# unneon/bioseqdb

Hardware: NVIDIA B200
Metric: 150bp_reads_aligned_per_sec (higher is better)
Workload: dtype int32

## Files before the change

bioseqdb_b200/csrc/finalize.cu:

```cuda
#include "pipeline.cuh"
#include <algorithm>
#include <cstdlib>
#include "ksw_warp.cuh"
#include "ksort_dev.cuh"
#include "launch_cache.cuh"

namespace {

constexpr int FIN_THREADS = 128;
constexpr int FIN_WARPS = FIN_THREADS / 32;
constexpr int NARROW_NC = 64;
constexpr int NARROW_TMAX = 192;
constexpr int NARROW_QMAX = 160;
constexpr int NARROW_THREADS = 128;
constexpr int NARROW_CIG = 48;

struct NarrowJob { uint32_t r, slot; int32_t w2, last_sc, it, score; };

struct FScratch { int* ehh; int* ehe; uint8_t* rseq; uint8_t* query; uint8_t* z; uint32_t* cig; };

__device__ __forceinline__ uint64_t hash_64(uint64_t key) {
    key += ~(key << 32); key ^= (key >> 22); key += ~(key << 13); key ^= (key >> 8);
    key += (key << 3); key ^= (key >> 15); key += ~(key << 27); key ^= (key >> 31);
    return key;
// ... 107 lines not shown
    r = (double)(a.re - b.rb) / (double)(b.re - a.rb) - (double)(a.qe - b.qb) / (double)(b.qe - a.qb);
    r = r > 0. ? r : -r;
    if (a.re < b.rb || a.qe < b.qb) {
        if (w > o.w << 1 || r >= (double)0.05f) return 0;
    } else if (w > o.w << 2 || r >= (double)(0.05f * 2)) return 0;
    w += a.w + b.w;
    w = w < o.w << 2 ? w : o.w << 2;
    GenOut g = gen_cigar2<false>(ix, o, smat, w, b.qe - a.qb, query + a.qb, a.rb, b.re, S, rseq_cap, 0, 0, overflow, need_rseq, cells, calls);
    score = g.score;
    q_s = (int)((double)(b.qe - a.qb) / (double)((b.qe - b.qb) + (a.qe - a.qb)) * (double)(b.score + a.score) + .499);
    r_s = (int)((double)(b.re - a.rb) / (double)((b.re - b.rb) + (a.re - a.rb)) * (double)(b.score + a.score) + .499);
    if ((double)score / (double)(q_s > r_s ? q_s : r_s) < (double)0.90f) return 0;
    *_w = w;
    return score;
}

__device__ __forceinline__ RowDev row_from_reg(const RegRec& ar, const int64_t* ann_id) {
    RowDev row;
    row.rb = ar.rb; row.re = ar.re; row.pos = 0; row.hash = ar.hash; row.qb = ar.qb; row.qe = ar.qe; row.rid = ar.rid; row.score = ar.score;
    row.truesc = ar.truesc; row.sub = ar.sub; row.csub = ar.csub; row.sub_n = ar.sub_n; row.w = ar.w; row.seedcov = ar.seedcov;
    row.secondary = ar.secondary; row.seedlen0 = ar.seedlen0; row.n_comp = ar.n_comp; row.frac_rep = ar.frac_rep;
    row.is_rev = 0; row.mapq = 0;
    row.NM = -1; row.flag = ar.secondary >= 0 ? 0x100 : 0; row.cigar_off = 0; row.n_cigar = 0;
    row.ref_id = ann_id[ar.rid];
    return row;
}

__device__ __forceinline__ int reg2aln_w2(const DevOpts& o, const RegRec& ar) {
    const int qb = ar.qb, qe = ar.qe; const int64_t rb = ar.rb, re = ar.re;
    int tmpw = infer_bw(qe - qb, (int)(re - rb), ar.truesc, o.a, o.o_del, o.e_del);
    int w2 = infer_bw(qe - qb, (int)(re - rb), ar.truesc, o.a, o.o_ins, o.e_ins);
    w2 = w2 > tmpw ? w2 : tmpw;
    if (w2 > o.w) w2 = w2 < ar.w ? w2 : ar.w;
    return w2;
}

__device__ __forceinline__ int gen_cigar_band(const DevOpts& o, int l_query, int rlen, int w_) {
    int max_ins = (int)((double)(((l_query + 1) >> 1) * o.mat[0] - o.o_ins) / o.e_ins + 1.);
    int max_del = (int)((double)(((l_query + 1) >> 1) * o.mat[0] - o.o_del) / o.e_del + 1.);
    int max_gap = max_ins > max_del ? max_ins : max_del;
    max_gap = max_gap > 1 ? max_gap : 1;
    int dl = rlen - l_query; dl = dl < 0 ? -dl : dl;
    int w = (max_gap + dl + 1) >> 1;
    w = w < w_ ? w : w_;
    const int min_w = dl + 3;
    return w > min_w ? w : min_w;
}

constexpr int REG_WT = 16;
constexpr uint32_t NARROW_SHORT_LIST = 1024;
constexpr int REG_WT3 = 8;
constexpr int REG_WT4 = 4;
constexpr int NARROW_T4_CNT = 20, NARROW_T8_CNT = 21;
constexpr int REG_WT2 = 32;
__device__ __forceinline__ bool narrow_is_big(const DevOpts& o, int lq, int rlen, int w2) {
    w2 = w2 < o.w << 2 ? w2 : o.w << 2;
    return gen_cigar_band(o, lq, rlen, w2) > REG_WT;
}
__device__ __forceinline__ bool narrow_is_tight(const DevOpts& o, int lq, int rlen, int wt = REG_WT3) {
    const int dl = lq - rlen;
    return (dl < 0 ? -dl : dl) <= wt && o.o_del >= 0 && o.e_del >= 0 && o.o_ins >= 0 && o.e_ins >= 0 && o.mat_max > 0;
}
__device__ __forceinline__ int narrow_class(const DevOpts& o, const RegRec& ar, uint32_t max_len) {
    const int lq = ar.qe - ar.qb; const int64_t rl = ar.re - ar.rb;
    if (max_len > NARROW_QMAX || lq <= 0 || rl <= 0 || rl > NARROW_TMAX) return 0;
    int w2 = reg2aln_w2(o, ar);
    w2 = w2 < o.w << 2 ? w2 : o.w << 2;
    if (lq == rl) return 2;
    if (2 * gen_cigar_band(o, lq, (int)rl, w2) + 1 <= NARROW_NC) return 1;
    return narrow_is_tight(o, lq, (int)rl) ? 1 : 0;
}
__device__ __forceinline__ void push_narrow(NarrowJob* list, uint32_t cap, uint32_t* cnt_reg, uint32_t* cnt_big, const NarrowJob& jb, bool big) {
    if (big) list[cap - 1u - atomicAdd(cnt_big, 1u)] = jb;
    else list[atomicAdd(cnt_reg, 1u)] = jb;
}

__device__ void reg2aln_warp(const FinalizeParams& P, const DevIndex& ix, const DevOpts& o, const int* smat, const FScratch& S, uint32_t cig_cap,
                             uint32_t rseq_cap, int l_query, const RegRec& ar, RowDev* out, unsigned long long& cells, unsigned long long& calls) {
    const int lane = lane_id();
    const int qb = ar.qb, qe = ar.qe; const int64_t rb = ar.rb, re = ar.re;
    int w2 = reg2aln_w2(o, ar);
    int it = 0, score = 0, last_sc = -(1 << 30);
    GenOut g;
    do {
        w2 = w2 < o.w << 2 ? w2 : o.w << 2;
        g = gen_cigar2<true>(ix, o, smat, w2, qe - qb, S.query + qb, rb, re, S, rseq_cap, P.z_cap, cig_cap - 2, P.overflow, P.need_rseq, cells, calls);
        if (g.ok) score = g.score;
        if (score == last_sc || w2 == o.w << 2) break;
        last_sc = score;
        w2 <<= 1;
    } while (++it < 3 && score < ar.truesc - o.a);
    int is_rev;
    int64_t pos = bns_depos(ix, rb < ix.l_pac ? rb : re - 1, &is_rev);
    int n_cigar = g.n_cigar, first = 0;
    if (n_cigar > 0) {
        if ((S.cig[0] & 0xf) == 2) { pos += S.cig[0] >> 4; first = 1; --n_cigar; }
        else if ((S.cig[g.n_cigar - 1] & 0xf) == 2) --n_cigar;
    }
    int clip5 = 0, clip3 = 0;
    if (qb != 0 || qe != l_query) { clip5 = is_rev ? l_query - qe : qb; clip3 = is_rev ? qb : l_query - qe; }
    const int n_out = n_cigar + (clip5 ? 1 : 0) + (clip3 ? 1 : 0);
    uint32_t coff = 0;
    if (lane == 0 && n_out) coff = atomicAdd(P.cigar_top, (uint32_t)n_out);
    coff = __shfl_sync(FULL, coff, 0);
    uint32_t r_off = 0, r_n = 0;
    if ((uint64_t)coff + (uint64_t)n_out > (uint64_t)P.cigar_cap) { if (lane == 0) atomicExch(P.overflow, 1u); }
// ... 166 lines not shown
            tmp = o.o_ins + o.e_ins > tmp ? o.o_ins + o.e_ins : tmp;
            int nz = 0;
            uint32_t* zl = S.cig;
            zl[nz++] = 0;
            for (int i = 1; i < n; ++i) {
                int k;
                for (k = 0; k < nz; ++k) {
                    const int j = (int)zl[k];
                    const int b_max = a[j].qb > a[i].qb ? a[j].qb : a[i].qb;
                    const int e_min = a[j].qe < a[i].qe ? a[j].qe : a[i].qe;
                    if (e_min > b_max) {
                        const int li = a[i].qe - a[i].qb, lj = a[j].qe - a[j].qb;
                        const int min_l = li < lj ? li : lj;
                        if ((float)(e_min - b_max) >= __fmul_rn((float)min_l, o.mask_level)) {
                            if (a[j].sub == 0) a[j].sub = a[i].score;
                            if (a[j].score - a[i].score <= tmp) ++a[j].sub_n;
                            break;
                        }
                    }
                }
                if (k == nz) { if ((uint32_t)nz < cig_cap) zl[nz] = (uint32_t)i; ++nz; }
                else a[i].secondary = (int)zl[k];
            }
            if ((uint32_t)nz > cig_cap) atomicExch(P.overflow, 2u);
        }
        __syncwarp();
        RowDev* rows = P.rows + blk.base;
        for (int i = 0; i < n; ++i) {
            const RegRec ar = a[i];
            RowDev row = row_from_reg(ar, P.ann_id);
            const int ncls = P.narrow_jobs != nullptr ? narrow_class(o, ar, P.max_len) : 0;
            const bool narrow = ncls != 0;
            if (lane == 0) {
                rows[i] = row;
                if (narrow) {
                    NarrowJob jb; jb.r = r; jb.slot = blk.base + i; jb.w2 = reg2aln_w2(o, ar); jb.last_sc = -(1 << 30); jb.it = 0; jb.score = 0;
                    NarrowJob* lists = reinterpret_cast<NarrowJob*>(P.narrow_jobs);
                    if (ncls == 1 && narrow_is_tight(o, ar.qe - ar.qb, (int)(ar.re - ar.rb))) {
                        if (narrow_is_tight(o, ar.qe - ar.qb, (int)(ar.re - ar.rb), REG_WT4)) lists[3u * P.narrow_cap + atomicAdd(P.narrow_cnt + NARROW_T4_CNT, 1u)] = jb;
                        else lists[4u * P.narrow_cap + atomicAdd(P.narrow_cnt + NARROW_T8_CNT, 1u)] = jb;
                    }
                    else if (ncls == 1) push_narrow(lists, P.narrow_cap, P.narrow_cnt, P.narrow_cnt + 5, jb, narrow_is_big(o, ar.qe - ar.qb, (int)(ar.re - ar.rb), jb.w2));
                    else lists[2u * P.narrow_cap + atomicAdd(P.narrow_cnt + 3, 1u)] = jb;
                }
            }
            __syncwarp();
            if (!narrow) reg2aln_warp(P, ix, o, smat, S, cig_cap, rseq_cap, l_query, ar, rows + i, cells, calls);
        }
        if (lane == 0) P.row_cnt[r] = (uint32_t)n;
    }
    if (P.counters && lane == 0) { atomicAdd(&P.counters[0], cells); atomicAdd(&P.counters[1], calls); }
}

template <int WT, bool TIGHT>
__device__ __forceinline__ int global_dp_reg(const uint8_t* __restrict__ qg, int lq, bool rev, const uint8_t* __restrict__ pac, int64_t tbase,
                                             int rlen, int w, int sA, int sB, int sN, int o_del, int e_del, int o_ins, int e_ins,
                                             uint32_t* __restrict__ Z, unsigned long long& cells, uint32_t* amb_out = nullptr) {
    uint32_t amb = 0;
    constexpr int W = 2 * WT + 1, NW = (W + 7) / 8, ZW = (W + 3) / 4;
    const int oe_del = o_del + e_del, oe_ins = o_ins + e_ins;
    int Hd[W], Ep[W + 1];
    uint32_t win[NW];
#pragma unroll
    for (int kk = 0; kk < W; ++kk) {
        const int j = kk - WT;
        Hd[kk] = (j >= 1 && j <= w) ? -(o_ins + e_ins * j) : KSW_NEG_INF;
        Ep[kk] = KSW_NEG_INF;
    }
    Ep[W] = KSW_NEG_INF;
#pragma unroll
    for (int x = 0; x < NW; ++x) win[x] = 0xffffffffu;
#pragma unroll
    for (int kk = WT; kk < W; ++kk) {
        const int j = kk - WT;
        if (j < lq) {
            const uint32_t b = rev ? qg[lq - 1 - j] : qg[j];
            amb |= b;
            win[kk >> 3] = (win[kk >> 3] & ~(15u << ((kk & 7) * 4))) | (b << ((kk & 7) * 4));
        }
    }
    int tb = rev ? 3 - (int)pac_get(pac, tbase) : (int)pac_get(pac, tbase);
    for (int i = 0; i < rlen; ++i) {
        const int beg = i > w ? i - w : 0;
        const int end = i + w + 1 < lq ? i + w + 1 : lq;
        const int ioff = i - WT - beg;
        const unsigned span = (unsigned)(end - beg);
        const int tz = beg == 0 ? 0 : 0x7fffffff;
        const int colm1 = i == 0 ? 0 : -(o_del + e_del * i);
        cells += span;
        int tb_next = 0; uint32_t nb = 15u;
        if (i + 1 < rlen) tb_next = rev ? 3 - (int)pac_get(pac, tbase + i + 1) : (int)pac_get(pac, tbase + i + 1);
        { const int jn = i + 1 + WT; if (jn < lq) { nb = rev ? qg[lq - 1 - jn] : qg[jn]; amb |= nb; } }
        int f = KSW_NEG_INF;
        uint32_t zpack = 0;
        uint32_t* zi = Z + (size_t)i * ZW * 32;
        if (TIGHT && w == WT && i > WT && i + WT + 1 <= lq) {
            uint32_t xw[NW];
#pragma unroll
            for (int x = 0; x < NW; ++x) xw[x] = win[x] ^ ((uint32_t)tb * 0x11111111u);
#pragma unroll
            for (int kk = 0; kk < W; ++kk) {
                const bool mis = ((xw[kk >> 3] >> ((kk & 7) * 4)) & 15u) != 0;
                const int m = Hd[kk] + (mis ? sB : sA);
                int e = Ep[kk + 1];
                int d = m >= e ? 0 : 1;
                int h = m >= e ? m : e;
// ... 1 lines not shown
                h = h >= f ? h : f;
                Hd[kk] = h;
                int tt = m - oe_del;
                e -= e_del;
                d |= e > tt ? 1 << 2 : 0;
                Ep[kk] = e > tt ? e : tt;
                tt = m - oe_ins;
                f -= e_ins;
                d |= f > tt ? 2 << 4 : 0;
                f = f > tt ? f : tt;
                zpack |= (uint32_t)d << ((kk & 3) * 8);
                if ((kk & 3) == 3 || kk == W - 1) { zi[(kk >> 2) * 32] = zpack; zpack = 0; }
            }
        } else
#pragma unroll
        for (int kk = 0; kk < W; ++kk) {
            const int t = ioff + kk;
            const bool valid = (unsigned)t < span;
            const int qb = (int)((win[kk >> 3] >> ((kk & 7) * 4)) & 15u);
            const int sc = qb == tb ? sA : (qb < 4 ? sB : sN);
            int m = (t == tz ? colm1 : Hd[kk]) + sc;
            int e = Ep[kk + 1];
            int d = m >= e ? 0 : 1;
            int h = m >= e ? m : e;
            d = h >= f ? d : 2;
            h = h >= f ? h : f;
            Hd[kk] = h;
            int tt = m - oe_del;
            e -= e_del;
            d |= e > tt ? 1 << 2 : 0;
            e = e > tt ? e : tt;
            Ep[kk] = valid ? e : KSW_NEG_INF;
            tt = m - oe_ins;
            int f2 = f - e_ins;
            d |= f2 > tt ? 2 << 4 : 0;
            f2 = f2 > tt ? f2 : tt;
            f = valid ? f2 : f;
            zpack |= (uint32_t)d << ((kk & 3) * 8);
            if ((kk & 3) == 3 || kk == W - 1) { zi[(kk >> 2) * 32] = zpack; zpack = 0; }
        }
#pragma unroll
        for (int x = 0; x + 1 < NW; ++x) win[x] = __funnelshift_r(win[x], win[x + 1], 4);
        win[NW - 1] = ((win[NW - 1] >> 4) & ~(15u << (((W - 1) & 7) * 4))) | (nb << (((W - 1) & 7) * 4));
        tb = tb_next;
    }
    const int ks = lq - rlen + WT;
    int score = KSW_NEG_INF;
#pragma unroll
    for (int kk = 0; kk < W; ++kk) if (kk == ks) score = Hd[kk];
    if (TIGHT && amb_out) *amb_out = amb;
    return score;
}

__device__ __forceinline__ uint32_t pac_win16(const uint8_t* pac, int64_t f) {
    const uint32_t* w = reinterpret_cast<const uint32_t*>(pac) + (f >> 4);
    return __funnelshift_l(__byte_perm(w[1], 0, 0x0123), __byte_perm(w[0], 0, 0x0123), (int)(f & 15) << 1);
}
__device__ __forceinline__ int diag_mismatches(const uint8_t* qg, int lq, bool rev, const uint8_t* pac, int64_t tbase, bool* ok) {
    const uint32_t* qa = reinterpret_cast<const uint32_t*>(reinterpret_cast<uintptr_t>(qg) & ~(uintptr_t)3);
    const int sh = (int)(reinterpret_cast<uintptr_t>(qg) & 3) * 8;
    uint32_t prev = qa[0], amb = 0;
    int mm = 0, j0 = 0;
    for (; j0 + 16 <= lq; j0 += 16) {
        uint32_t Q = 0;
#pragma unroll
        for (int k = 0; k < 4; ++k) {
            const uint32_t nx = qa[(j0 >> 2) + k + 1];
            const uint32_t x = __funnelshift_r(prev, nx, sh);
            prev = nx;
            amb |= x;
            Q |= ((x | x >> 6 | x >> 12 | x >> 18) & 0xffu) << (8 * k);
        }
        uint32_t v;
        if (rev) v = ~pac_win16(pac, tbase + lq - 16 - j0);
        else {
            const uint32_t r = __brev(pac_win16(pac, tbase + j0));
            v = ((r >> 1) & 0x55555555u) | ((r & 0x55555555u) << 1);
        }
        const uint32_t d = Q ^ v;
        mm += __popc((d | d >> 1) & 0x55555555u);
    }
    for (int j = j0; j < lq; ++j) {
        const uint32_t q = qg[j];
        amb |= q;
        mm += q != (rev ? 3u - pac_get(pac, tbase + lq - 1 - j) : pac_get(pac, tbase + j));
    }
    *ok = (amb & 0xfcfcfcfcu) == 0;
    return mm;
}

struct NarrowParams {
    const uint8_t* seqs; const uint64_t* offs; const RegRec* regs; RowDev* rows;
    const NarrowJob* jobs; int job_stride; const uint32_t* n_jobs;
    NarrowJob* requeue; uint32_t requeue_cap; uint32_t* requeue_cnt; uint32_t* requeue_big_cnt; uint64_t* wide_jobs; uint32_t* wide_cnt;
    uint32_t* cigar_pool; uint32_t cigar_cap; uint32_t* cigar_top;
    uint8_t* zbuf; uint32_t* ticket; uint32_t* overflow; unsigned long long* counters;
    NarrowJob* tight; uint32_t* tight_cnt;
    uint32_t short_list;
};

template <int MODE>
__global__ void __launch_bounds__(NARROW_THREADS, MODE == 5 ? 10 : (MODE >= 3 ? 6 : (MODE == 1 ? 4 : 2))) regs_cigar_narrow(NarrowParams P, DevIndex ix, DevOpts o) {
    __shared__ int smat[25];
    if (threadIdx.x < 25) smat[threadIdx.x] = o.mat[threadIdx.x];
    __syncthreads();
    const int tid = threadIdx.x, lane = tid & 31;
    const uint32_t gwarp = (blockIdx.x * NARROW_THREADS + tid) >> 5;
    constexpr int WTM = MODE == 2 ? REG_WT2 : (MODE == 3 ? REG_WT3 : (MODE == 4 ? REG_WT4 : REG_WT));
    constexpr int ZROW = (2 * WTM + 1 + 3) / 4;
    uint32_t* Z = reinterpret_cast<uint32_t*>(P.zbuf + (size_t)gwarp * NARROW_TMAX * ZROW * 4 * 32) + lane;
    int oe_del = o.o_del + o.e_del, oe_ins = o.o_ins + o.e_ins, e_del = o.e_del, e_ins = o.e_ins;
    asm volatile("" : "+r"(oe_del), "+r"(oe_ins), "+r"(e_del), "+r"(e_ins));
    const int64_t l_pac = ix.l_pac;
    const uint32_t n_jobs = *P.n_jobs;
    constexpr bool diag_pass = MODE == 5;
    const bool short_list = !diag_pass && n_jobs <= P.short_list;
    unsigned long long cells = 0, calls = 0;
    for (;;) {
        uint32_t t = next_ticket(P.ticket);
        if ((uint64_t)t * 32 >= n_jobs) break;
        const uint32_t j_id = t * 32 + lane;
        uint32_t cg[NARROW_CIG];
        int e_nc = 0, e_first = 0, e_clip5 = 0, e_clip3 = 0, e_n = 0;
        uint32_t e_slot = 0; bool e_on = false;
        if (j_id < n_jobs) {
            const NarrowJob jb = P.jobs[(long)j_id * P.job_stride];
            const uint32_t r = jb.r, slot = jb.slot;
            const uint64_t job = (uint64_t)r << 32 | slot;
            const RegRec ar = P.regs[slot];
            const int l_read = (int)(P.offs[r + 1] - P.offs[r]);
            const int qb = ar.qb, qe = ar.qe, lq = qe - qb;
            const int64_t rb = ar.rb, re = ar.re;
            const int rlen = (int)(re - rb);
            const bool rev = rb >= l_pac;
            const bool reject = lq <= 0 || rb >= re || (rb < l_pac && re > l_pac) || rb < 0 || re > (l_pac << 1);
            const int64_t tbase = rev ? (l_pac << 1) - re : rb;
            const uint8_t* qg = P.seqs + P.offs[r] + qb;
            auto qat = [&](int j) -> int { return (int)(rev ? qg[lq - 1 - j] : qg[j]); };
            int n_cigar = 0, NM = -1, score = jb.score;
            int w2 = jb.w2 < o.w << 2 ? jb.w2 : o.w << 2;
            bool go_wide = false, again = false;
            do {
                n_cigar = 0; NM = -1;
                if (short_list && !reject) { go_wide = true; break; }
                int nm_known = -1;
                if (!reject) {
                    bool diagonal = lq == rlen && w2 == 0;
                    if (diag_pass && lq == rlen) {
                        int sc = 0;
                        bool fast = false;
                        const int mm = diag_mismatches(qg, lq, rev, ix.pac, tbase, &fast);
                        if (fast) { sc = smat[0] * (lq - mm) + smat[1] * mm; nm_known = mm; }
// ... 88 lines not shown
                }
            } while (false);
            if (go_wide) {
                uint32_t k = atomicAdd(P.wide_cnt, 1u);
                P.wide_jobs[k] = job;
            } else if (!again) {
                int is_rev;
                int64_t pos = bns_depos(ix, rb < l_pac ? rb : re - 1, &is_rev);
                int nc = n_cigar, first = 0;
                if (nc > 0) {
                    if ((cg[0] & 0xf) == 2) { pos += cg[0] >> 4; first = 1; --nc; }
                    else if ((cg[n_cigar - 1] & 0xf) == 2) --nc;
                }
                int clip5 = 0, clip3 = 0;
                if (qb != 0 || qe != l_read) { clip5 = is_rev ? l_read - qe : qb; clip3 = is_rev ? qb : l_read - qe; }
                e_nc = nc; e_first = first; e_clip5 = clip5; e_clip3 = clip3; e_n = nc + (clip5 ? 1 : 0) + (clip3 ? 1 : 0);
                e_slot = slot; e_on = true;
                RowDev* out = P.rows + slot;
                const int rid = bns_pos2rid(ix, pos);
                out->NM = NM; out->is_rev = is_rev; out->pos = pos - ix.ann_offset[rid < 0 ? 0 : rid];
            }
        }
        __syncwarp();
        {
            uint32_t incl = (uint32_t)e_n;
#pragma unroll
            for (int d = 1; d < 32; d <<= 1) { const uint32_t up = __shfl_up_sync(FULL, incl, d); if (lane >= d) incl += up; }
            uint32_t base = 0;
            if (lane == 31 && incl) base = atomicAdd(P.cigar_top, incl);
            base = __shfl_sync(FULL, base, 31);
            if (e_on) {
                const uint32_t coff = base + incl - (uint32_t)e_n;
                RowDev* out = P.rows + e_slot;
                if ((uint64_t)coff + (uint64_t)e_n > (uint64_t)P.cigar_cap) { atomicExch(P.overflow, 1u); }
                else {
                    uint32_t* dst = P.cigar_pool + coff;
                    int k = 0;
                    if (e_clip5) dst[k++] = (uint32_t)e_clip5 << 4 | 3;
                    for (int c = 0; c < e_nc; ++c) dst[k++] = cg[e_first + c];
                    if (e_clip3) dst[k++] = (uint32_t)e_clip3 << 4 | 3;
                    out->cigar_off = coff; out->n_cigar = (uint32_t)e_n;
                }
            }
        }
        __syncwarp();
    }
    if (P.counters) {
        cells = __reduce_add_sync(FULL, (unsigned)(cells & 0xffffffffu)) + ((unsigned long long)__reduce_add_sync(FULL, (unsigned)(cells >> 32)) << 32);
        calls = __reduce_add_sync(FULL, (unsigned)calls);
        if (lane == 0) { atomicAdd(&P.counters[0], cells); atomicAdd(&P.counters[1], calls); }
    }
}

template <bool SMEM>
__global__ void __launch_bounds__(FIN_THREADS) regs_cigar_wide(FinalizeParams P, DevIndex ix, DevOpts o, uint32_t cig_cap, uint32_t rseq_cap) {
    extern __shared__ __align__(16) uint8_t dyn_smem[];
    __shared__ int smat[25];
    if (threadIdx.x < 25) smat[threadIdx.x] = o.mat[threadIdx.x];
    __syncthreads();
    const int lane = lane_id();
    const uint32_t gwarp = (blockIdx.x * FIN_THREADS + threadIdx.x) >> 5;
    FScratch S;
    {
        const size_t fast = ((size_t)(P.max_len + 2) * 8 + rseq_cap + P.max_len + 15) & ~(size_t)15;
        uint8_t* gbase = P.scratch + (size_t)gwarp * P.scratch_per_warp;
        uint8_t* fbase = SMEM ? dyn_smem + (size_t)(threadIdx.x >> 5) * fast : gbase;
        S.ehh = reinterpret_cast<int*>(fbase);
        S.ehe = S.ehh + (P.max_len + 2);
        S.rseq = reinterpret_cast<uint8_t*>(S.ehe + (P.max_len + 2));
        S.query = S.rseq + rseq_cap;
        S.cig = reinterpret_cast<uint32_t*>(gbase + fast);
        S.z = reinterpret_cast<uint8_t*>(S.cig + cig_cap);
    }
    unsigned long long cells = 0, calls = 0;
    const uint32_t n_jobs = *P.wide_cnt;
    for (;;) {
        uint32_t t = next_ticket(P.ticket);
        if (t >= n_jobs) break;
        const uint64_t job = P.wide_jobs[t];
        const uint32_t r = (uint32_t)(job >> 32), slot = (uint32_t)job;
        const int l_query = (int)(P.offs[r + 1] - P.offs[r]);
        const uint8_t* qg = P.seqs + P.offs[r];
        for (int i = lane; i < l_query; i += 32) S.query[i] = qg[i];
        __syncwarp();
        const RegRec ar = P.regs[slot];
        reg2aln_warp(P, ix, o, smat, S, cig_cap, rseq_cap, l_query, ar, P.rows + slot, cells, calls);
    }
    if (P.counters && lane == 0) { atomicAdd(&P.counters[0], cells); atomicAdd(&P.counters[1], calls); }
}

}

static size_t fin_fast_bytes(uint32_t max_len, uint32_t rseq_cap) { return ((size_t)(max_len + 2) * 8 + rseq_cap + max_len + 15) & ~(size_t)15; }
static uint32_t fin_cig_cap(uint32_t max_len, uint32_t rseq_cap) { return max_len + rseq_cap + 8; }

size_t finalize_scratch_per_warp(uint32_t max_len, uint32_t rseq_cap, uint32_t* z_cap_out) {
    uint64_t z = (uint64_t)max_len * (uint64_t)rseq_cap;
    const uint64_t z_band = (uint64_t)rseq_cap * 1024;
    if (z > z_band) z = z_band;
    if (z_cap_out) *z_cap_out = (uint32_t)z;
    size_t b = fin_fast_bytes(max_len, rseq_cap) + (size_t)fin_cig_cap(max_len, rseq_cap) * 4 + (size_t)z;
    return (b + 255) & ~(size_t)255;
}

static bool fin_use_smem(uint32_t max_len, uint32_t rseq_cap) { return fin_fast_bytes(max_len, rseq_cap) * FIN_WARPS <= 40 * 1024; }

int finalize_resident_warps() {
    return cached_blocks_per_sm(regs_finalize<false>, FIN_THREADS, 0) * cached_sm_count() * FIN_WARPS;
}

template <int MODE> static int narrow_blocks() { return cached_blocks_per_sm(regs_cigar_narrow<MODE>, NARROW_THREADS, 0) * cached_sm_count(); }
static size_t narrow_z_bytes(int blocks, int wt) { return (size_t)blocks * (NARROW_THREADS / 32) * NARROW_TMAX * ((2 * wt + 1 + 3) / 4) * 4 * 32; }
static size_t narrow_z_front() {
    return std::max(narrow_z_bytes(narrow_blocks<1>(), REG_WT), std::max(narrow_z_bytes(narrow_blocks<3>(), REG_WT3), narrow_z_bytes(narrow_blocks<4>(), REG_WT4)));
}

size_t narrow_zbuf_bytes() { return narrow_z_front() + narrow_z_bytes(narrow_blocks<2>(), REG_WT2); }

void launch_finalize(const FinalizeParams& p, const DevIndex& ix, const DevOpts& o, cudaStream_t st, uint32_t rseq_cap, int n_warps, uint64_t* launches, const ExtAux* aux) {
    const uint32_t cig_cap = fin_cig_cap(p.max_len, rseq_cap);
    int blocks = n_warps / FIN_WARPS;
    if (blocks < 1) blocks = 1;
    const bool smem_ok = fin_use_smem(p.max_len, rseq_cap);
    const size_t smem = smem_ok ? fin_fast_bytes(p.max_len, rseq_cap) * FIN_WARPS : 0;
    if (p.todo && p.narrow_jobs && p.n_reads) {
        regs_finalize_thread<<<(p.n_reads + 127) / 128, 128, 0, st>>>(p, ix, o);
        if (launches) ++*launches;
    }
    if (smem_ok) regs_finalize<true><<<blocks, FIN_THREADS, smem, st>>>(p, ix, o, cig_cap, rseq_cap);
    else regs_finalize<false><<<blocks, FIN_THREADS, 0, st>>>(p, ix, o, cig_cap, rseq_cap);
    if (launches) ++*launches;
    if (!p.narrow_jobs) return;
    {
        NarrowJob* listA = reinterpret_cast<NarrowJob*>(p.narrow_jobs);
        NarrowJob* listB = listA + p.narrow_cap;
        NarrowJob* listS = listA + 2 * (size_t)p.narrow_cap;
        NarrowJob* listT4 = listA + 3 * (size_t)p.narrow_cap;
        NarrowJob* listT8 = listA + 4 * (size_t)p.narrow_cap;
        for (int pass = 0; pass < 4; ++pass) {
            NarrowParams q;
            q.seqs = p.seqs; q.offs = p.offs; q.regs = p.regs; q.rows = p.rows;
            NarrowJob* in = pass == 0 ? listS : (pass == 2 ? listB : listA);
            q.requeue = (pass == 0 || pass == 2) ? listA : listB; q.requeue_cap = p.narrow_cap;
            q.requeue_cnt = p.narrow_cnt + (pass == 0 ? 0 : (pass == 1 ? 1 : (pass == 2 ? 2 : 4)));
            q.requeue_big_cnt = p.narrow_cnt + (pass == 0 ? 5 : (pass == 1 ? 6 : (pass == 2 ? 7 : 4)));
            q.wide_jobs = p.wide_jobs; q.wide_cnt = p.wide_cnt; q.cigar_pool = p.cigar_pool; q.cigar_cap = p.cigar_cap; q.cigar_top = p.cigar_top;
            q.zbuf = p.narrow_z; q.overflow = p.overflow; q.counters = p.counters;
            q.tight = listT4; q.tight_cnt = p.narrow_cnt + NARROW_T4_CNT;
            { static const uint32_t sl = getenv("BSQ_FIN_SHORT_LIST") ? (uint32_t)atoi(getenv("BSQ_FIN_SHORT_LIST")) : NARROW_SHORT_LIST; q.short_list = sl; }
            q.jobs = in; q.job_stride = 1; q.ticket = p.ticket + 1 + pass;
            q.n_jobs = p.narrow_cnt + (pass == 0 ? 3 : (pass == 1 ? 0 : (pass == 2 ? 1 : 2)));
            if (pass == 0) {
                regs_cigar_narrow<5><<<narrow_blocks<5>(), NARROW_THREADS, 0, st>>>(q, ix, o);
                q.jobs = listT4; q.n_jobs = p.narrow_cnt + NARROW_T4_CNT; q.ticket = p.ticket + 9;
                q.tight = listT8; q.tight_cnt = p.narrow_cnt + NARROW_T8_CNT;
                regs_cigar_narrow<4><<<narrow_blocks<4>(), NARROW_THREADS, 0, st>>>(q, ix, o);
                q.jobs = listT8; q.n_jobs = p.narrow_cnt + NARROW_T8_CNT; q.ticket = p.ticket + 10;
                regs_cigar_narrow<3><<<narrow_blocks<3>(), NARROW_THREADS, 0, st>>>(q, ix, o);
                if (launches) *launches += 3;
            } else {
                cudaStream_t s2 = aux ? aux->st[0] : st;
                if (aux) { cudaEventRecord(aux->ev[0], st); cudaStreamWaitEvent(s2, aux->ev[0], 0); }
                regs_cigar_narrow<1><<<narrow_blocks<1>(), NARROW_THREADS, 0, st>>>(q, ix, o);
                q.jobs = in + p.narrow_cap - 1; q.job_stride = -1; q.ticket = p.ticket + 5 + pass;
                q.n_jobs = p.narrow_cnt + (pass == 1 ? 5 : (pass == 2 ? 6 : 7));
                q.zbuf = p.narrow_z + narrow_z_front();
                regs_cigar_narrow<2><<<narrow_blocks<2>(), NARROW_THREADS, 0, s2>>>(q, ix, o);
                if (aux) { cudaEventRecord(aux->ev[1], s2); cudaStreamWaitEvent(st, aux->ev[1], 0); }
                if (launches) *launches += 2;
            }
        }
    }
    {
        FinalizeParams w = p;
        w.ticket = p.ticket + 5;
        if (smem_ok) regs_cigar_wide<true><<<blocks, FIN_THREADS, smem, st>>>(w, ix, o, cig_cap, rseq_cap);
        else regs_cigar_wide<false><<<blocks, FIN_THREADS, 0, st>>>(w, ix, o, cig_cap, rseq_cap);
        if (launches) ++*launches;
    }
}
```

Before: 63.02 million.

## Pack two tight banded DP jobs per thread using 16-bit SIMD lanes

Adds a paired tight-pass kernel in which each thread runs the banded global DP for two jobs at once. The H/E/F values are packed as int16x2 and updated with __viaddmax/__vibmax SIMD intrinsics, and edge rows fall back to a scalar per-half path. The aim is to roughly halve the per-job instruction count in the tight WT=4 and WT=8 passes. In exchange it doubles the traceback buffer per lane, adds a range check that falls back to the old kernel when scores might overflow 16 bits, and adds register pressure plus divergence from mismatched job lengths.

```diff
diff --git a/bioseqdb_b200/csrc/finalize.cu b/bioseqdb_b200/csrc/finalize.cu
--- a/bioseqdb_b200/csrc/finalize.cu
+++ b/bioseqdb_b200/csrc/finalize.cu
@@ -183,6 +183,7 @@
 constexpr int REG_WT3 = 8;
 constexpr int REG_WT4 = 4;
 constexpr int NARROW_T4_CNT = 20, NARROW_T8_CNT = 21;
+constexpr int NARROW_PAIR_CNT = 22;
 constexpr int REG_WT2 = 32;
 __device__ __forceinline__ bool narrow_is_big(const DevOpts& o, int lq, int rlen, int w2) {
     w2 = w2 < o.w << 2 ? w2 : o.w << 2;
@@ -455,6 +456,98 @@
     if (P.counters && lane == 0) { atomicAdd(&P.counters[0], cells); atomicAdd(&P.counters[1], calls); }
 }
 
+template <int WT, bool TIGHT, int ZS>
+__device__ __forceinline__ void dp_row(int (&Hd)[2 * WT + 1], int (&Ep)[2 * WT + 2], const uint32_t (&win)[(2 * WT + 8) / 8], int tb, int i,
+                                       int lq, int w, int sA, int sB, int sN, int o_del, int e_del, int e_ins, int oe_del, int oe_ins, int neg,
+                                       uint32_t* __restrict__ zi, unsigned long long& cells) {
+    constexpr int W = 2 * WT + 1, NW = (W + 7) / 8;
+    const int beg = i > w ? i - w : 0;
+    const int end = i + w + 1 < lq ? i + w + 1 : lq;
+    const int ioff = i - WT - beg;
+    const unsigned span = (unsigned)(end - beg);
+    const int tz = beg == 0 ? 0 : 0x7fffffff;
+    const int colm1 = i == 0 ? 0 : -(o_del + e_del * i);
+    cells += span;
+    int f = neg;
+    uint32_t zpack = 0;
+    if (TIGHT && w == WT && i > WT && i + WT + 1 <= lq) {
+        uint32_t xw[NW];
+#pragma unroll
+        for (int x = 0; x < NW; ++x) xw[x] = win[x] ^ ((uint32_t)tb * 0x11111111u);
+#pragma unroll
+        for (int kk = 0; kk < W; ++kk) {
+            const bool mis = ((xw[kk >> 3] >> ((kk & 7) * 4)) & 15u) != 0;
+            const int m = Hd[kk] + (mis ? sB : sA);
+            int e = Ep[kk + 1];
+            int d = m >= e ? 0 : 1;
+            int h = m >= e ? m : e;
+            d = h >= f ? d : 2;
+            h = h >= f ? h : f;
+            Hd[kk] = h;
+            int tt = m - oe_del;
+            e -= e_del;
+            d |= e > tt ? 1 << 2 : 0;
+            Ep[kk] = e > tt ? e : tt;
+            tt = m - oe_ins;
+            f -= e_ins;
+            d |= f > tt ? 2 << 4 : 0;
+            f = f > tt ? f : tt;
+            zpack |= (uint32_t)d << ((kk & 3) * 8);
+            if ((kk & 3) == 3 || kk == W - 1) { zi[(kk >> 2) * ZS] = zpack; zpack = 0; }
+        }
+    } else
+#pragma unroll
+    for (int kk = 0; kk < W; ++kk) {
+        const int t = ioff + kk;
+        const bool valid = (unsigned)t < span;
+        const int qb = (int)((win[kk >> 3] >> ((kk & 7) * 4)) & 15u);
+        const int sc = qb == tb ? sA : (qb < 4 ? sB : sN);
+        int m = (t == tz ? colm1 : Hd[kk]) + sc;
+        int e = Ep[kk + 1];
+        int d = m >= e ? 0 : 1;
+        int h = m >= e ? m : e;
+        d = h >= f ? d : 2;
+        h = h >= f ? h : f;
+        Hd[kk] = h;
+        int tt = m - oe_del;
+        e -= e_del;
+        d |= e > tt ? 1 << 2 : 0;
+        e = e > tt ? e : tt;
+        Ep[kk] = valid ? e : neg;
+        tt = m - oe_ins;
+        int f2 = f - e_ins;
+        d |= f2 > tt ? 2 << 4 : 0;
+        f2 = f2 > tt ? f2 : tt;
+        f = valid ? f2 : f;
+        zpack |= (uint32_t)d << ((kk & 3) * 8);
+        if ((kk & 3) == 3 || kk == W - 1) { zi[(kk >> 2) * ZS] = zpack; zpack = 0; }
+    }
+}
+
+template <int WT>
+__device__ __forceinline__ void window_init(uint32_t (&win)[(2 * WT + 8) / 8], const uint8_t* __restrict__ qg, int lq, bool rev, uint32_t& amb) {
+    constexpr int W = 2 * WT + 1, NW = (W + 7) / 8;
+#pragma unroll
+    for (int x = 0; x < NW; ++x) win[x] = 0xffffffffu;
+#pragma unroll
+    for (int kk = WT; kk < W; ++kk) {
+        const int j = kk - WT;
+        if (j < lq) {
+            const uint32_t b = rev ? qg[lq - 1 - j] : qg[j];
+            amb |= b;
+            win[kk >> 3] = (win[kk >> 3] & ~(15u << ((kk & 7) * 4))) | (b << ((kk & 7) * 4));
+        }
+    }
+}
+
+template <int WT>
+__device__ __forceinline__ void window_slide(uint32_t (&win)[(2 * WT + 8) / 8], uint32_t nb) {
+    constexpr int W = 2 * WT + 1, NW = (W + 7) / 8;
+#pragma unroll
+    for (int x = 0; x + 1 < NW; ++x) win[x] = __funnelshift_r(win[x], win[x + 1], 4);
+    win[NW - 1] = ((win[NW - 1] >> 4) & ~(15u << (((W - 1) & 7) * 4))) | (nb << (((W - 1) & 7) * 4));
+}
+
 template <int WT, bool TIGHT>
 __device__ __forceinline__ int global_dp_reg(const uint8_t* __restrict__ qg, int lq, bool rev, const uint8_t* __restrict__ pac, int64_t tbase,
                                              int rlen, int w, int sA, int sB, int sN, int o_del, int e_del, int o_ins, int e_ins,
@@ -562,6 +655,133 @@
     return score;
 }
 
+constexpr int PAIR_NEG = -0x4000;
+
+struct DpHalf { const uint8_t* qg; int64_t tbase; int lq, rlen, w; bool rev; };
+
+__device__ __forceinline__ uint32_t prmt(uint32_t a, uint32_t b, uint32_t sel) {
+    uint32_t r;
+    asm("prmt.b32 %0, %1, %2, %3;" : "=r"(r) : "r"(a), "r"(b), "r"(sel));
+    return r;
+}
+__device__ __forceinline__ uint32_t pk2(int v) { return ((uint32_t)v & 0xffffu) * 0x10001u; }
+
+template <int WT>
+__device__ __noinline__ unsigned pair_edge_row(uint32_t* __restrict__ st, int h, const uint32_t (&win)[(2 * WT + 8) / 8], int tb, int i, int lq, int w,
+                                               int sA, int sB, int sN, int o_del, int e_del, int o_ins, int e_ins, uint32_t* __restrict__ zi) {
+    constexpr int W = 2 * WT + 1;
+    const int sh = 16 * h;
+    int H[W], E[W + 1];
+#pragma unroll
+    for (int kk = 0; kk < W; ++kk) { H[kk] = (int16_t)(st[kk] >> sh); E[kk] = (int16_t)(st[W + kk] >> sh); }
+    E[W] = PAIR_NEG;
+    unsigned long long cells = 0;
+    dp_row<WT, true, 64>(H, E, win, tb, i, lq, w, sA, sB, sN, o_del, e_del, e_ins, o_del + e_del, o_ins + e_ins, PAIR_NEG, zi, cells);
+#pragma unroll
+    for (int kk = 0; kk < W; ++kk) {
+        st[kk] = h ? __byte_perm(st[kk], (uint32_t)H[kk], 0x5410) : __byte_perm((uint32_t)H[kk], st[kk], 0x7610);
+        st[W + kk] = h ? __byte_perm(st[W + kk], (uint32_t)E[kk], 0x5410) : __byte_perm((uint32_t)E[kk], st[W + kk], 0x7610);
+    }
+    return (unsigned)cells;
+}
+
+template <int WT>
+__device__ __noinline__ void global_dp_reg_pair(const DpHalf (&hf)[2], const uint8_t* __restrict__ pac, int sA, int sB, int sN, int o_del, int e_del,
+                                                   int o_ins, int e_ins, uint32_t* __restrict__ Z, unsigned long long& cells, int (&score)[2], uint32_t (&amb)[2]) {
+    constexpr int W = 2 * WT + 1, NW = (W + 7) / 8, ZW = (W + 3) / 4;
+    const int oe_del = o_del + e_del, oe_ins = o_ins + e_ins;
+    const uint32_t n_oe_del = pk2(-oe_del), n_oe_ins = pk2(-oe_ins), n_e_del = pk2(-e_del), n_e_ins = pk2(-e_ins), lo = 0x80008000u;
+    const uint32_t t_lo = ((uint32_t)sA & 0xffu) | ((uint32_t)sB & 0xffu) * 0x01010100u, t_hi = ((uint32_t)sB & 0xffu) * 0x01010101u;
+    uint32_t Hd[W], Ep[W + 1];
+    uint32_t win[2][NW];
+    int tb[2];
+#pragma unroll
+    for (int kk = 0; kk < W; ++kk) {
+        const int j = kk - WT;
+        const int a = (j >= 1 && j <= hf[0].w) ? -(o_ins + e_ins * j) : PAIR_NEG, b = (j >= 1 && j <= hf[1].w) ? -(o_ins + e_ins * j) : PAIR_NEG;
+        Hd[kk] = ((uint32_t)a & 0xffffu) | (uint32_t)b << 16;
+        Ep[kk] = pk2(PAIR_NEG);
+    }
+    Ep[W] = pk2(PAIR_NEG);
+#pragma unroll
+    for (int h = 0; h < 2; ++h) {
+        amb[h] = 0; score[h] = KSW_NEG_INF;
+        window_init<WT>(win[h], hf[h].qg, hf[h].rlen > 0 ? hf[h].lq : 0, hf[h].rev, amb[h]);
+        tb[h] = hf[h].rlen > 0 ? (hf[h].rev ? 3 - (int)pac_get(pac, hf[h].tbase) : (int)pac_get(pac, hf[h].tbase)) : 0;
+    }
+    const int rows = hf[0].rlen > hf[1].rlen ? hf[0].rlen : hf[1].rlen;
+    for (int i = 0; i < rows; ++i) {
+        bool live[2], tight[2];
+        int tb_next[2]; uint32_t nb[2];
+#pragma unroll
+        for (int h = 0; h < 2; ++h) {
+            const DpHalf& d = hf[h];
+            live[h] = i < d.rlen;
+            tight[h] = live[h] && d.w == WT && i > WT && i + WT + 1 <= d.lq;
+            tb_next[h] = 0; nb[h] = 15u;
+            if (i + 1 < d.rlen) tb_next[h] = d.rev ? 3 - (int)pac_get(pac, d.tbase + i + 1) : (int)pac_get(pac, d.tbase + i + 1);
+            const int jn = i + 1 + WT;
+            if (live[h] && jn < d.lq) { nb[h] = d.rev ? d.qg[d.lq - 1 - jn] : d.qg[jn]; amb[h] |= nb[h]; }
+        }
+        uint32_t* zi = Z + (size_t)i * ZW * 64;
+        if ((tight[0] || !live[0]) && (tight[1] || !live[1])) {
+            uint32_t sb[2][ZW];
+#pragma unroll
+            for (int h = 0; h < 2; ++h) {
+                uint32_t xw[NW];
+#pragma unroll
+                for (int x = 0; x < NW; ++x) xw[x] = win[h][x] ^ ((uint32_t)tb[h] * 0x11111111u);
+#pragma unroll
+                for (int g = 0; g < ZW; ++g) sb[h][g] = prmt(t_lo, t_hi, (g & 1) ? xw[g >> 1] >> 16 : xw[g >> 1]);
+            }
+            uint32_t f = pk2(PAIR_NEG), za = 0, zb = 0;
+#pragma unroll
+            for (int kk = 0; kk < W; ++kk) {
+                const uint32_t p = (uint32_t)(kk & 3);
+                const uint32_t sc = prmt(sb[0][kk >> 2], sb[1][kk >> 2], p | (p | 8u) << 4 | (p + 4u) << 8 | (p + 12u) << 12);
+                const uint32_t m = __viaddmax_s16x2(Hd[kk], sc, lo);
+                const uint32_t e = Ep[kk + 1];
+                bool mh, ml, fh, fl, eh, el, gh, gl;
+                uint32_t hh = __vibmax_s16x2(m, e, &mh, &ml);
+                hh = __vibmax_s16x2(hh, f, &fh, &fl);
+                Hd[kk] = hh;
+                Ep[kk] = __vibmax_s16x2(__viaddmax_s16x2(m, n_oe_del, lo), __viaddmax_s16x2(e, n_e_del, lo), &eh, &el);
+                f = __vibmax_s16x2(__viaddmax_s16x2(m, n_oe_ins, lo), __viaddmax_s16x2(f, n_e_ins, lo), &gh, &gl);
+                const uint32_t da = (fl ? (ml ? 0u : 1u) : 2u) | (el ? 0u : 4u) | (gl ? 0u : 32u);
+                const uint32_t db = (fh ? (mh ? 0u : 1u) : 2u) | (eh ? 0u : 4u) | (gh ? 0u : 32u);
+                za |= da << ((kk & 3) * 8);
+                zb |= db << ((kk & 3) * 8);
+                if ((kk & 3) == 3 || kk == W - 1) { reinterpret_cast<uint2*>(zi)[(kk >> 2) * 32] = make_uint2(za, zb); za = 0; zb = 0; }
+            }
+            cells += (live[0] ? W : 0) + (live[1] ? W : 0);
+        } else {
+            uint32_t st[2 * W];
+#pragma unroll
+            for (int kk = 0; kk < W; ++kk) { st[kk] = Hd[kk]; st[W + kk] = Ep[kk]; }
+#pragma unroll
+            for (int h = 0; h < 2; ++h) {
+                if (!live[h]) continue;
+                uint32_t wh[NW];
+#pragma unroll
+                for (int x = 0; x < NW; ++x) wh[x] = win[h][x];
+                cells += pair_edge_row<WT>(st, h, wh, tb[h], i, hf[h].lq, hf[h].w, sA, sB, sN, o_del, e_del, o_ins, e_ins, zi + h);
+            }
+#pragma unroll
+            for (int kk = 0; kk < W; ++kk) { Hd[kk] = st[kk]; Ep[kk] = st[W + kk]; }
+        }
+#pragma unroll
+        for (int h = 0; h < 2; ++h) {
+            if (i == hf[h].rlen - 1) {
+                const int ks = hf[h].lq - hf[h].rlen + WT;
+#pragma unroll
+                for (int kk = 0; kk < W; ++kk) if (kk == ks) score[h] = (int16_t)(Hd[kk] >> (16 * h));
+            }
+            if (live[h]) window_slide<WT>(win[h], nb[h]);
+            tb[h] = tb_next[h];
+        }
+    }
+}
+
 __device__ __forceinline__ uint32_t pac_win16(const uint8_t* pac, int64_t f) {
     const uint32_t* w = reinterpret_cast<const uint32_t*>(pac) + (f >> 4);
     return __funnelshift_l(__byte_perm(w[1], 0, 0x0123), __byte_perm(w[0], 0, 0x0123), (int)(f & 15) << 1);
@@ -607,7 +827,178 @@
     uint8_t* zbuf; uint32_t* ticket; uint32_t* overflow; unsigned long long* counters;
     NarrowJob* tight; uint32_t* tight_cnt;
     uint32_t short_list;
+    uint32_t* pair_passes;
 };
+
+__host__ __device__ constexpr int narrow_wt(int mode) { return mode == 2 ? REG_WT2 : (mode == 3 ? REG_WT3 : (mode == 4 ? REG_WT4 : REG_WT)); }
+
+struct NarrowTry {
+    NarrowJob jb; RegRec ar;
+    const uint8_t* qg; int64_t tbase;
+    int l_read, lq, rlen, w2, wx, w, score, n_cigar, NM, nm_known;
+    bool rev, reject, stop, dp, go_wide, again;
+};
+struct PoolEntry { int nc, first, clip5, clip3, n; uint32_t slot; bool on; };
+
+__device__ __forceinline__ int narrow_qat(const NarrowTry& T, int j) { return (int)(T.rev ? T.qg[T.lq - 1 - j] : T.qg[j]); }
+
+template <int MODE>
+__device__ __forceinline__ void narrow_begin(const NarrowParams& P, const DevIndex& ix, const DevOpts& o, const int* smat, bool short_list, int oe_del,
+                                             int oe_ins, const NarrowJob& jb, uint32_t (&cg)[NARROW_CIG], NarrowTry& T) {
+    constexpr bool diag_pass = MODE == 5;
+    constexpr int WTM = narrow_wt(MODE);
+    const int64_t l_pac = ix.l_pac;
+    const uint32_t r = jb.r;
+    T.jb = jb;
+    T.ar = P.regs[jb.slot];
+    T.l_read = (int)(P.offs[r + 1] - P.offs[r]);
+    const int qb = T.ar.qb, lq = T.ar.qe - qb;
+    const int64_t rb = T.ar.rb, re = T.ar.re;
+    const int rlen = (int)(re - rb);
+    T.lq = lq; T.rlen = rlen;
+    T.rev = rb >= l_pac;
+    T.reject = lq <= 0 || rb >= re || (rb < l_pac && re > l_pac) || rb < 0 || re > (l_pac << 1);
+    T.tbase = T.rev ? (l_pac << 1) - re : rb;
+    T.qg = P.seqs + P.offs[r] + qb;
+    T.n_cigar = 0; T.NM = -1; T.score = jb.score; T.nm_known = -1;
+    T.w2 = jb.w2 < o.w << 2 ? jb.w2 : o.w << 2;
+    T.wx = T.w = 0;
+    T.stop = T.dp = T.go_wide = T.again = false;
+    if (short_list && !T.reject) { T.go_wide = true; T.stop = true; return; }
+    if (T.reject) return;
+    bool diagonal = lq == rlen && T.w2 == 0;
+    if (diag_pass && lq == rlen) {
+        int sc = 0;
+        bool fast = false;
+        const int mm = diag_mismatches(T.qg, lq, T.rev, ix.pac, T.tbase, &fast);
+        if (fast) { sc = smat[0] * (lq - mm) + smat[1] * mm; T.nm_known = mm; }
+        else for (int i = 0; i < lq; ++i) {
+            const int tb = T.rev ? 3 - (int)pac_get(ix.pac, T.tbase + i) : (int)pac_get(ix.pac, T.tbase + i);
+            sc += smat[tb * 5 + narrow_qat(T, i)];
+        }
+        if (diagonal || sc > (lq - 1) * o.mat_max - oe_ins - oe_del) { T.score = sc; cg[0] = (uint32_t)lq << 4; T.n_cigar = 1; diagonal = true; }
+        else {
+            if (narrow_is_tight(o, lq, rlen)) P.tight[atomicAdd(P.tight_cnt, 1u)] = jb;
+            else push_narrow(P.requeue, P.requeue_cap, P.requeue_cnt, P.requeue_big_cnt, jb, narrow_is_big(o, lq, rlen, jb.w2));
+            T.again = true; T.stop = true; return;
+        }
+    } else if (diagonal) {
+        int sc = 0;
+        for (int i = 0; i < lq; ++i) {
+            const int tb = T.rev ? 3 - (int)pac_get(ix.pac, T.tbase + i) : (int)pac_get(ix.pac, T.tbase + i);
+            sc += smat[tb * 5 + narrow_qat(T, i)];
+        }
+        T.score = sc; cg[0] = (uint32_t)lq << 4; T.n_cigar = 1;
+    }
+    if (MODE != 5 && !diagonal) {
+        const int wx = gen_cigar_band(o, lq, rlen, T.w2);
+        const int w = MODE >= 3 ? (wx < WTM ? wx : WTM) : wx;
+        T.wx = wx; T.w = w;
+        if (MODE >= 3 && (!narrow_is_tight(o, lq, rlen, WTM) || rlen > NARROW_TMAX)) {
+            push_narrow(P.requeue, P.requeue_cap, P.requeue_cnt, P.requeue_big_cnt, jb, narrow_is_big(o, lq, rlen, jb.w2));
+            T.again = true; T.stop = true; return;
+        }
+        if (MODE < 3 && (w > WTM || rlen > NARROW_TMAX)) { T.go_wide = true; T.stop = true; return; }
+        T.dp = true;
+    }
+}
+
+template <int MODE, int ZS>
+__device__ __forceinline__ void narrow_end(const NarrowParams& P, const DevIndex& ix, const DevOpts& o, int e_del, int e_ins, NarrowTry& T,
+                                           uint32_t (&cg)[NARROW_CIG], uint32_t amb, const uint32_t* __restrict__ Zr, PoolEntry& pe) {
+    constexpr bool diag_pass = MODE == 5;
+    constexpr int WTM = narrow_wt(MODE);
+    constexpr int ZROW = (2 * WTM + 1 + 3) / 4;
+    const int64_t l_pac = ix.l_pac;
+    const NarrowJob& jb = T.jb;
+    const int lq = T.lq, rlen = T.rlen;
+    int n_cigar = T.n_cigar;
+    do {
+        if (T.stop) break;
+        if (T.dp) {
+            const int w = T.w, wx = T.wx;
+            if (MODE >= 3 && (amb & ~3u)) {
+                push_narrow(P.requeue, P.requeue_cap, P.requeue_cnt, P.requeue_big_cnt, jb, narrow_is_big(o, lq, rlen, jb.w2));
+                T.again = true; break;
+            }
+            if (MODE >= 3 && w < wx) {
+                const int k = w + 1, dl = lq - rlen;
+                const int ubp = o.mat_max * (lq - k) - (o.o_ins + e_ins * k) - (o.o_del + e_del * (k - dl));
+                const int ubm = o.mat_max * (rlen - k) - (o.o_del + e_del * k) - (o.o_ins + e_ins * (k + dl));
+                if (T.score <= (ubp > ubm ? ubp : ubm)) {
+                    if (MODE == 4) P.tight[atomicAdd(P.tight_cnt, 1u)] = jb;
+                    else push_narrow(P.requeue, P.requeue_cap, P.requeue_cnt, P.requeue_big_cnt, jb, narrow_is_big(o, lq, rlen, jb.w2));
+                    T.again = true; break;
+                }
+            }
+            int which = 0, i = rlen - 1, k = (i + w + 1 < lq ? i + w + 1 : lq) - 1;
+            bool full = false;
+            auto push = [&](uint32_t op, uint32_t len) {
+                if (n_cigar == 0 || op != (cg[n_cigar - 1] & 0xf)) { if (n_cigar < NARROW_CIG) cg[n_cigar++] = len << 4 | op; else full = true; }
+                else cg[n_cigar - 1] += len << 4;
+            };
+            while (i >= 0 && k >= 0) {
+                const int jj = k - i + WTM;
+                which = (int)(Zr[((size_t)i * ZROW + (jj >> 2)) * ZS] >> ((jj & 3) << 3) & 0xff) >> (which << 1) & 3;
+                if (which == 0) { push(0, 1); --i; --k; }
+                else if (which == 1) { push(2, 1); --i; }
+                else { push(1, 1); --k; }
+            }
+            if (i >= 0) push(2, (uint32_t)(i + 1));
+            if (k >= 0) push(1, (uint32_t)(k + 1));
+            if (full) { T.go_wide = true; break; }
+            for (int a = 0; a < n_cigar >> 1; ++a) { uint32_t x = cg[a]; cg[a] = cg[n_cigar - 1 - a]; cg[n_cigar - 1 - a] = x; }
+        }
+        if (!T.reject) {
+            int x = 0, y = 0, n_mm = 0, n_gap = 0;
+            if (T.nm_known >= 0 && n_cigar == 1) n_mm = T.nm_known;
+            else for (int k = 0; k < n_cigar; ++k) {
+                const int op = (int)(cg[k] & 0xf), len = (int)(cg[k] >> 4);
+                if (op == 0) {
+                    bool fast = false;
+                    int mm = 0;
+                    if (len >= 16) mm = diag_mismatches(T.rev ? T.qg + (lq - x - len) : T.qg + x, len, T.rev, ix.pac, T.tbase + y, &fast);
+                    if (fast) n_mm += mm;
+                    else for (int i = 0; i < len; ++i) {
+                        const int tb = T.rev ? 3 - (int)pac_get(ix.pac, T.tbase + y + i) : (int)pac_get(ix.pac, T.tbase + y + i);
+                        n_mm += narrow_qat(T, x + i) != tb;
+                    }
+                    x += len; y += len;
+                } else if (op == 2) { if (k > 0 && k < n_cigar - 1) n_gap += len; y += len; }
+                else if (op == 1) { x += len; n_gap += len; }
+            }
+            T.NM = n_mm + n_gap;
+        }
+        if (T.score == jb.last_sc || T.w2 == o.w << 2) break;
+        if (diag_pass && !T.reject && lq == rlen && !(lq == rlen && T.w2 == 0)) break;
+        if (jb.it + 1 < 3 && T.score < T.ar.truesc - o.a) {
+            T.again = true;
+            NarrowJob nx; nx.r = jb.r; nx.slot = jb.slot; nx.w2 = T.w2 << 1; nx.last_sc = T.score; nx.it = jb.it + 1; nx.score = T.score;
+            push_narrow(P.requeue, P.requeue_cap, P.requeue_cnt, P.requeue_big_cnt, nx, narrow_is_big(o, lq, rlen, nx.w2));
+        }
+    } while (false);
+    pe.on = false; pe.n = 0;
+    if (T.go_wide) {
+        uint32_t k = atomicAdd(P.wide_cnt, 1u);
+        P.wide_jobs[k] = (uint64_t)jb.r << 32 | jb.slot;
+    } else if (!T.again) {
+        const int qb = T.ar.qb, qe = T.ar.qe; const int64_t rb = T.ar.rb, re = T.ar.re;
+        int is_rev;
+        int64_t pos = bns_depos(ix, rb < l_pac ? rb : re - 1, &is_rev);
+        int nc = n_cigar, first = 0;
+        if (nc > 0) {
+            if ((cg[0] & 0xf) == 2) { pos += cg[0] >> 4; first = 1; --nc; }
+            else if ((cg[n_cigar - 1] & 0xf) == 2) --nc;
+        }
+        int clip5 = 0, clip3 = 0;
+        if (qb != 0 || qe != T.l_read) { clip5 = is_rev ? T.l_read - qe : qb; clip3 = is_rev ? qb : T.l_read - qe; }
+        pe.nc = nc; pe.first = first; pe.clip5 = clip5; pe.clip3 = clip3; pe.n = nc + (clip5 ? 1 : 0) + (clip3 ? 1 : 0);
+        pe.slot = jb.slot; pe.on = true;
+        RowDev* out = P.rows + jb.slot;
+        const int rid = bns_pos2rid(ix, pos);
+        out->NM = T.NM; out->is_rev = is_rev; out->pos = pos - ix.ann_offset[rid < 0 ? 0 : rid];
+    }
+}
 
 template <int MODE>
 __global__ void __launch_bounds__(NARROW_THREADS, MODE == 5 ? 10 : (MODE >= 3 ? 6 : (MODE == 1 ? 4 : 2))) regs_cigar_narrow(NarrowParams P, DevIndex ix, DevOpts o) {
@@ -802,6 +1193,96 @@
     }
 }
 
+template <int MODE>
+__global__ void __launch_bounds__(NARROW_THREADS, 6) regs_cigar_tight_pair(NarrowParams P, DevIndex ix, DevOpts o) {
+    static_assert(MODE == 3 || MODE == 4, "pairs run the tight passes only");
+    __shared__ int smat[25];
+    if (threadIdx.x < 25) smat[threadIdx.x] = o.mat[threadIdx.x];
+    __syncthreads();
+    const int tid = threadIdx.x, lane = tid & 31;
+    const uint32_t gwarp = (blockIdx.x * NARROW_THREADS + tid) >> 5;
+    constexpr int NH = 2;
+    constexpr int WTM = narrow_wt(MODE);
+    constexpr int ZROW = (2 * WTM + 1 + 3) / 4;
+    uint32_t* Z = reinterpret_cast<uint32_t*>(P.zbuf + (size_t)gwarp * NARROW_TMAX * ZROW * 4 * 32 * NH) + lane * NH;
+    int oe_del = o.o_del + o.e_del, oe_ins = o.o_ins + o.e_ins, e_del = o.e_del, e_ins = o.e_ins;
+    asm volatile("" : "+r"(oe_del), "+r"(oe_ins), "+r"(e_del), "+r"(e_ins));
+    const uint32_t n_jobs = *P.n_jobs;
+    if (blockIdx.x == 0 && tid == 0) atomicAdd(P.pair_passes, 1u);
+    const bool short_list = n_jobs <= P.short_list;
+    unsigned long long cells = 0, calls = 0;
+    for (;;) {
+        uint32_t t = next_ticket(P.ticket);
+        if ((uint64_t)t * 32 * NH >= n_jobs) break;
+        uint32_t cg[NH][NARROW_CIG];
+        NarrowTry T[NH];
+        PoolEntry pe[NH];
+        uint32_t amb[NH];
+        bool on[NH];
+#pragma unroll
+        for (int h = 0; h < NH; ++h) {
+            const uint32_t j_id = (t * 32 + lane) * NH + h;
+            on[h] = j_id < n_jobs;
+            amb[h] = 0; pe[h].on = false; pe[h].n = 0;
+            if (on[h]) narrow_begin<MODE>(P, ix, o, smat, short_list, oe_del, oe_ins, P.jobs[(long)j_id * P.job_stride], cg[h], T[h]);
+        }
+        {
+            DpHalf hf[2];
+            bool any = false;
+#pragma unroll
+            for (int h = 0; h < 2; ++h) {
+                const bool dp = on[h] && T[h].dp;
+                any |= dp; calls += dp;
+                hf[h] = dp ? DpHalf{T[h].qg, T[h].tbase, T[h].lq, T[h].rlen, T[h].w, T[h].rev} : DpHalf{nullptr, 0, 0, 0, 0, false};
+            }
+            if (any) {
+                int sc[2];
+                global_dp_reg_pair<WTM>(hf, ix.pac, smat[0], smat[1], smat[4], o.o_del, e_del, o.o_ins, e_ins, Z, cells, sc, amb);
+#pragma unroll
+                for (int h = 0; h < 2; ++h) if (on[h] && T[h].dp) T[h].score = sc[h];
+            }
+        }
+#pragma unroll
+        for (int h = 0; h < NH; ++h) if (on[h]) narrow_end<MODE, 32 * NH>(P, ix, o, e_del, e_ins, T[h], cg[h], amb[h], Z + h, pe[h]);
+        __syncwarp();
+        {
+            uint32_t n_lane = 0;
+#pragma unroll
+            for (int h = 0; h < NH; ++h) n_lane += (uint32_t)pe[h].n;
+            uint32_t incl = n_lane;
+#pragma unroll
+            for (int d = 1; d < 32; d <<= 1) { const uint32_t up = __shfl_up_sync(FULL, incl, d); if (lane >= d) incl += up; }
+            uint32_t base = 0;
+            if (lane == 31 && incl) base = atomicAdd(P.cigar_top, incl);
+            base = __shfl_sync(FULL, base, 31);
+            uint32_t coff = base + incl - n_lane;
+#pragma unroll
+            for (int h = 0; h < NH; ++h) {
+                const PoolEntry& e = pe[h];
+                if (e.on) {
+                    RowDev* out = P.rows + e.slot;
+                    if ((uint64_t)coff + (uint64_t)e.n > (uint64_t)P.cigar_cap) { atomicExch(P.overflow, 1u); }
+                    else {
+                        uint32_t* dst = P.cigar_pool + coff;
+                        int k = 0;
+                        if (e.clip5) dst[k++] = (uint32_t)e.clip5 << 4 | 3;
+                        for (int c = 0; c < e.nc; ++c) dst[k++] = cg[h][e.first + c];
+                        if (e.clip3) dst[k++] = (uint32_t)e.clip3 << 4 | 3;
+                        out->cigar_off = coff; out->n_cigar = (uint32_t)e.n;
+                    }
+                }
+                coff += (uint32_t)e.n;
+            }
+        }
+        __syncwarp();
+    }
+    if (P.counters) {
+        cells = __reduce_add_sync(FULL, (unsigned)(cells & 0xffffffffu)) + ((unsigned long long)__reduce_add_sync(FULL, (unsigned)(cells >> 32)) << 32);
+        calls = __reduce_add_sync(FULL, (unsigned)calls);
+        if (lane == 0) { atomicAdd(&P.counters[0], cells); atomicAdd(&P.counters[1], calls); }
+    }
+}
+
 template <bool SMEM>
 __global__ void __launch_bounds__(FIN_THREADS) regs_cigar_wide(FinalizeParams P, DevIndex ix, DevOpts o, uint32_t cig_cap, uint32_t rseq_cap) {
     extern __shared__ __align__(16) uint8_t dyn_smem[];
@@ -860,9 +1341,19 @@
 }
 
 template <int MODE> static int narrow_blocks() { return cached_blocks_per_sm(regs_cigar_narrow<MODE>, NARROW_THREADS, 0) * cached_sm_count(); }
-static size_t narrow_z_bytes(int blocks, int wt) { return (size_t)blocks * (NARROW_THREADS / 32) * NARROW_TMAX * ((2 * wt + 1 + 3) / 4) * 4 * 32; }
+template <int MODE> static int pair_blocks() { return cached_blocks_per_sm(regs_cigar_tight_pair<MODE>, NARROW_THREADS, 0) * cached_sm_count(); }
+static size_t narrow_z_bytes(int blocks, int wt, int per_lane = 1) { return (size_t)blocks * (NARROW_THREADS / 32) * NARROW_TMAX * ((2 * wt + 1 + 3) / 4) * 4 * 32 * per_lane; }
 static size_t narrow_z_front() {
-    return std::max(narrow_z_bytes(narrow_blocks<1>(), REG_WT), std::max(narrow_z_bytes(narrow_blocks<3>(), REG_WT3), narrow_z_bytes(narrow_blocks<4>(), REG_WT4)));
+    size_t b = narrow_z_bytes(narrow_blocks<1>(), REG_WT);
+    b = std::max(b, std::max(narrow_z_bytes(narrow_blocks<3>(), REG_WT3), narrow_z_bytes(narrow_blocks<4>(), REG_WT4)));
+    return std::max(b, std::max(narrow_z_bytes(pair_blocks<3>(), REG_WT3, 2), narrow_z_bytes(pair_blocks<4>(), REG_WT4, 2)));
+}
+
+static bool tight_pairs_fit(const DevOpts& o, int wt) {
+    int64_t S = 0;
+    for (int k = 0; k < 25; ++k) S = std::max<int64_t>(S, o.mat[k] < 0 ? -(int64_t)o.mat[k] : o.mat[k]);
+    const int64_t O = std::max(o.o_del, o.o_ins), E = std::max(o.e_del, o.e_ins);
+    return S <= 127 && 2 * O + (wt + 2) * E + S * (NARROW_QMAX + 1) < -PAIR_NEG && PAIR_NEG - E >= -0x8000;
 }
 
 size_t narrow_zbuf_bytes() { return narrow_z_front() + narrow_z_bytes(narrow_blocks<2>(), REG_WT2); }
@@ -896,7 +1387,7 @@
             q.requeue_big_cnt = p.narrow_cnt + (pass == 0 ? 5 : (pass == 1 ? 6 : (pass == 2 ? 7 : 4)));
             q.wide_jobs = p.wide_jobs; q.wide_cnt = p.wide_cnt; q.cigar_pool = p.cigar_pool; q.cigar_cap = p.cigar_cap; q.cigar_top = p.cigar_top;
             q.zbuf = p.narrow_z; q.overflow = p.overflow; q.counters = p.counters;
-            q.tight = listT4; q.tight_cnt = p.narrow_cnt + NARROW_T4_CNT;
+            q.tight = listT4; q.tight_cnt = p.narrow_cnt + NARROW_T4_CNT; q.pair_passes = p.narrow_cnt + NARROW_PAIR_CNT;
             { static const uint32_t sl = getenv("BSQ_FIN_SHORT_LIST") ? (uint32_t)atoi(getenv("BSQ_FIN_SHORT_LIST")) : NARROW_SHORT_LIST; q.short_list = sl; }
             q.jobs = in; q.job_stride = 1; q.ticket = p.ticket + 1 + pass;
             q.n_jobs = p.narrow_cnt + (pass == 0 ? 3 : (pass == 1 ? 0 : (pass == 2 ? 1 : 2)));
@@ -904,9 +1395,11 @@
                 regs_cigar_narrow<5><<<narrow_blocks<5>(), NARROW_THREADS, 0, st>>>(q, ix, o);
                 q.jobs = listT4; q.n_jobs = p.narrow_cnt + NARROW_T4_CNT; q.ticket = p.ticket + 9;
                 q.tight = listT8; q.tight_cnt = p.narrow_cnt + NARROW_T8_CNT;
-                regs_cigar_narrow<4><<<narrow_blocks<4>(), NARROW_THREADS, 0, st>>>(q, ix, o);
+                if (tight_pairs_fit(o, REG_WT4)) regs_cigar_tight_pair<4><<<pair_blocks<4>(), NARROW_THREADS, 0, st>>>(q, ix, o);
+                else regs_cigar_narrow<4><<<narrow_blocks<4>(), NARROW_THREADS, 0, st>>>(q, ix, o);
                 q.jobs = listT8; q.n_jobs = p.narrow_cnt + NARROW_T8_CNT; q.ticket = p.ticket + 10;
-                regs_cigar_narrow<3><<<narrow_blocks<3>(), NARROW_THREADS, 0, st>>>(q, ix, o);
+                if (tight_pairs_fit(o, REG_WT3)) regs_cigar_tight_pair<3><<<pair_blocks<3>(), NARROW_THREADS, 0, st>>>(q, ix, o);
+                else regs_cigar_narrow<3><<<narrow_blocks<3>(), NARROW_THREADS, 0, st>>>(q, ix, o);
                 if (launches) *launches += 3;
             } else {
                 cudaStream_t s2 = aux ? aux->st[0] : st;
```

Result: slower. 59.97 million, median of 6 (-4.8%).
